# Kotstantinovskiy/SonicDiffusionBayesLab

Measured on AMD Instinct MI355X. Metric: 512x512 images/sec at 50 DDIM steps, higher is better.
Workload: dtype bf16; 1 GPU; SD-1.5 512x512 DDIM 50 steps, CFG 7.5, batch=8/GPU (BASELINE configs[1]); global_batch=8, sample_size=64, parallelism=batch-shard x1, weights=SD-1.5-shaped synthetic seed 1234

## Files before the change

include/sd_hip.h:

```cpp
#ifndef SD_HIP_H
#define SD_HIP_H

#ifdef __cplusplus
extern "C" {
#endif

typedef struct sd_unet sd_unet;

typedef struct sd_unet_config {
    int sample_size;
    int in_channels;
    int out_channels;
    int num_levels;
    int block_out_channels[8];
    int layers_per_block;
    int attn_levels[8];
    int cross_attention_dim;
    int num_heads;
    int norm_num_groups;
    float norm_eps;
    int context_len;
    int weight_dtype;
    float fp8_act_scale_norm;
    float fp8_act_scale_ff;
// ... 126 lines not shown
int sd_unet_debug_tensor(sd_unet* u, void* stream, const char* name, float* host_out, long long numel,
                         void* workspace, int unet_batch, int cache_branch_id);

int sd_sched_step(void* stream, const float* eps, int cfg, float guidance, const float* x, const float* m1,
                  const float* m2, const float* m3, const float* noise, float* prev, float* y2, float* m_out,
                  const float coef[10], long long n);

int sd_cfg_rescale_factors(void* stream, const float* eps, int batch, long long n_per_sample, float guidance,
                           float rescale, float* k_out);
int sd_sched_step_rescaled(void* stream, const float* eps, int cfg, float guidance, const float* x, const float* m1,
                           const float* m2, const float* m3, const float* noise, float* prev, float* y2, float* m_out,
                           const float coef[10], long long n, const float* k, long long n_per_sample);

int sd_sched_step_inpaint(void* stream, const float* eps, int cfg, float guidance, const float* x, const float* m1,
                          const float* m2, const float* m3, const float* noise, float* prev, float* y2, float* m_out,
                          const float coef[10], long long n, const float* k, long long n_per_sample, const float* init,
                          const float* blend_noise, const float* mask, float a, float s, long long hw);
int sd_inpaint_prepare(void* stream, const float* image, const float* mask, float* masked_image, float* latent_mask,
                       int batch, int height, int width);

int sd_op_gemm(void* stream, const void* X, long long ldx, const void* X2, long long ldx2, int K1, const void* W,
               const float* bias, const float* bias2, const void* R, long long ldr, void* C, long long ldc, int M,
               int N, int K, int epi);
int sd_op_gemm_batched(void* stream, const void* X, long long ldx, const void* W, long long w_batch_stride,
                       int rows_per_batch, const float* bias, const void* R, long long ldr, void* C, long long ldc,
                       int M, int N, int K, int epi, int sm_valid);
int sd_op_gemm_batched_softmax_ln(void* stream, const void* X, long long ldx, const void* W, long long w_batch_stride,
                                  int rows_per_batch, void* C, long long ldc, int M, int N, int K, int sm_valid,
                                  const float* rowstats, int parts, const float* c1, const float* c2, float eps);
int sd_op_conv3x3(void* stream, const void* X, const void* W, const float* bias, const float* bias2, const void* R,
                  void* Y, int B, int Hin, int Win, int Cin, int Cout, int stride, int upsample);
int sd_op_conv3x3_shortcut(void* stream, const void* X, const void* W, const float* bias, const void* Xs1, int Cs1,
                           const void* Xs2, int Cs2, const void* Wsc, void* Y, int B, int H, int Wd, int Cin, int Cout);
int sd_op_conv3x3_shortcut_groupnorm(void* stream, const void* X, const void* W, const float* bias, const void* Xs1, int Cs1,
                                     const void* Xs2, int Cs2, const void* Wsc, void* Y, int B, int H, int Wd, int Cin,
                                     int Cout, const float* gamma, const float* beta, void* Yn, int groups, float eps, int silu);
int sd_op_conv3x3_down_asym(void* stream, const void* X, const void* W, const float* bias, void* Y, int B, int Hin, int Win,
                            int Cin, int Cout);
int sd_op_conv3x3_kernel(int M, int N, int Cin, int Hin, int Win, int stride, int upsample, int dtype);
int sd_op_softmax_rows(void* stream, void* S, long long rows, int cols, float scale);
int sd_op_conv3x3_upsample_subpixel(void* stream, const void* X, const void* W4, const float* bias, void* Y, int B, int Hin,
                                    int Win, int Cin, int Cout);
int sd_op_conv3x3_upsample_subpixel_groupnorm(void* stream, const void* X, const void* W4, const float* bias, void* Y, int B,
                                              int Hin, int Win, int Cin, int Cout, const float* gamma, const float* beta,
                                              void* Yn, int groups, float eps, int silu);
int sd_op_groupnorm(void* stream, const void* x1, int C1, const void* x2, int C2, const float* gamma,
                    const float* beta, void* y, int B, int HW, int groups, float eps, int silu);
int sd_op_conv3x3_groupnorm(void* stream, const void* X, const void* W, const float* bias, const float* bias2,
                            const void* R, void* Y, int B, int Hin, int Win, int Cin, int Cout, const float* gamma,
                            const float* beta, void* Yn, int groups, float eps, int silu);
int sd_op_conv3x3_splitk(int M, int Cout, int Cin, int Hin, int Win, int stride, int upsample);
int sd_op_layernorm(void* stream, const void* x, const float* gamma, const float* beta, void* y, int rows, int C,
                    float eps);
int sd_op_attention(void* stream, const void* Q, long long ldq, const void* K, long long ldk, const void* V,
                    long long ldv, void* O, long long ldo, int B, int heads, int Nq, int Nk, int D, float scale);
int sd_op_gemm_qkv_headmajor(void* stream, const void* X, long long ldx, const void* W, void* Q, void* KV, int M, int C,
                             int tokens, int K);
int sd_op_attention_headmajor(void* stream, const void* Q, long long ldq, const void* K, const void* V, void* O,
                              long long ldo, int B, int heads, int Nq, int Nk, int D, float scale);
int sd_op_clip_attention(void* stream, const void* qkv, void* out, int B, int L, int H, int heads);
int sd_op_vit_attention(void* stream, const void* qkv, void* out, int B, int L, int H, int heads);
int sd_op_clip_preprocess(void* stream, const unsigned char* images, int B, int H, int W, int S, int P, unsigned char* crop,
                          void* patches);
int sd_op_conv_in(void* stream, const float* x, int Bsrc, const float* Wt, const float* bias, void* y, int B, int H,
                  int W, int Cin, int Cout);
int sd_op_conv_in_cond(void* stream, const float* x, int Bsrc, const float* cond, int Bcond, const float* Wt,
                       const float* bias, void* y, int B, int H, int W, int Cout);
int sd_op_conv_out(void* stream, const void* x, const void* Wp, const float* bias, float* y, int B, int H, int W,
                   int Cin, int Cout);
int sd_op_time_embedding(void* stream, float t, const void* W1, const float* b1, const void* W2, const float* b2,
                         float* scratch, float* temb, int dim_in, int dim);
int sd_op_timestep_cond(void* stream, float t, const float* cond, const void* Wc, float* row, float* emb, int cond_dim,
                        int dim);

int sd_op_ln_partials(int kind, int M, int N);
int sd_op_gemm_rowstats(void* stream, const void* X, long long ldx, const void* W, const float* bias, const void* R,
                        long long ldr, void* C, long long ldc, int M, int N, int K, float* rowstats);
int sd_op_gemm_ln(void* stream, const void* X, long long ldx, const void* Wg, const float* c1, const float* c2,
                  const float* rowstats, int parts, float eps, void* C, long long ldc, int M, int N, int K, int epi);
int sd_op_gemm_plan(void* stream, const void* X, long long ldx, const void* X2, long long ldx2, int K1, const void* W,
                    const float* bias, const float* bias2, const void* R, long long ldr, void* C, long long ldc, int M, int N,
                    int K, float* rowstats, float* stats, const float* ln_rs, int ln_parts, const float* ln_c1, float ln_eps,
                    void* KV, int hm_tokens);
int sd_op_xattn_fused_rowstats(void* stream, const void* X, const void* R, void* Y, const void* At, const void* Bw,
                               const float* bias, int M, int C, int rows_per_sample, int L, float* rowstats);
int sd_op_xattn_fused(void* stream, const void* X, const void* R, void* Y, const void* At, const void* Bw,
                      const float* bias, int M, int C, int rows_per_sample, int L);
int sd_op_xattn_fused_ln(void* stream, const void* X, const void* R, void* Y, const void* At, const void* Bw,
                         const float* bias, int M, int C, int rows_per_sample, int L, const float* ln_rowstats, int ln_parts,
                         long long ln_rows, const float* c2, float eps, float* rowstats);
int sd_op_conv3x3_ablate(void* stream, const void* X, const void* W, void* Y, int B, int Hin, int Win, int Cin, int Cout,
                         int ablate);
int sd_op_xattn_fused_stamps(void* stream, const void* X, const void* R, void* Y, const void* At, const void* Bw,
                             const float* bias, int M, int C, int rows_per_sample, int L, unsigned long long* stamps);

int sd_op_gemm_fp8(void* stream, const void* X, long long ldx, const void* W, const float* wscale, float xscale,
                   const float* bias, const void* R, long long ldr, void* C, long long ldc, int M, int N, int K, int epi,
                   int out_fp8, float oscale);
int sd_op_conv3x3_fp8(void* stream, const void* X, const void* W, const float* wscale, float xscale, const float* bias,
                      const float* bias2, const void* R, void* Y, int B, int Hin, int Win, int Cin, int Cout, int stride,
                      int upsample);
int sd_op_groupnorm_fp8(void* stream, const void* x1, int C1, const void* x2, int C2, const float* gamma,
                        const float* beta, void* y, int B, int HW, int groups, float eps, int silu, int Cpad, float oscale);
int sd_op_layernorm_fp8(void* stream, const void* x, const float* gamma, const float* beta, void* y, int rows, int C,
                        int Cpad, float eps, float oscale);
int sd_op_quantize_fp8(void* stream, const void* x_bf16, void* y_fp8, long long rows, int C, int Cpad, float scale);
int sd_op_amax_e4m3(void* stream, const void* codes, long long nbytes, unsigned* out_code);

#ifdef __cplusplus
}
#endif
#endif
```

sonicdiffusionbayeslab_amd/_lib.py:

```python
from __future__ import annotations

import ctypes as C
import os
import re
from typing import Optional

HERE = os.path.dirname(os.path.abspath(__file__))
LIB_PATH = os.environ.get("SD_AMD_LIB", os.path.join(HERE, "lib", "libsdhip.so"))
HEADER_PATH = os.path.normpath(os.path.join(HERE, "..", "include", "sd_hip.h"))

ABLATE_LIB_PATH = os.path.join(HERE, "lib", "libsdhip_ablate.so")

_lib: Optional[C.CDLL] = None
_ablate: Optional[C.CDLL] = None


class SdUnetConfig(C.Structure):
    _fields_ = [
        ("sample_size", C.c_int), ("in_channels", C.c_int), ("out_channels", C.c_int),
        ("num_levels", C.c_int), ("block_out_channels", C.c_int * 8), ("layers_per_block", C.c_int),
        ("attn_levels", C.c_int * 8), ("cross_attention_dim", C.c_int), ("num_heads", C.c_int),
        ("norm_num_groups", C.c_int), ("norm_eps", C.c_float), ("context_len", C.c_int),
        ("weight_dtype", C.c_int), ("fp8_act_scale_norm", C.c_float), ("fp8_act_scale_ff", C.c_float),
        ("time_cond_proj_dim", C.c_int),
# ... 43 lines not shown
    "sd_unet_fp8_scale_count": (_i, [_vp]),
    "sd_unet_fp8_scale_info": (_i, [_vp, _i, C.c_char_p, _i, C.POINTER(_f), C.POINTER(_f)]),
    "sd_unet_set_fp8_scale": (_i, [_vp, C.c_char_p, _f]),
    "sd_unet_workspace_bytes": (_ll, [_vp, _i, _i]),
    "sd_unet_set_context": (_i, [_vp, _vp, _vp, _i, _i, _vp, _ll]),
    "sd_unet_set_timestep_cond": (_i, [_vp, _vp, _vp]),
    "sd_unet_forward": (_i, [_vp, _vp, _vp, _i, _i, _f, _vp, _vp, _ll, _i, _i]),
    "sd_unet_workspace_bytes_hw": (_ll, [_vp, _i, _i, _i, _i]),
    "sd_unet_set_context_hw": (_i, [_vp, _vp, _vp, _i, _i, _i, _i, _vp, _ll]),
    "sd_unet_forward_hw": (_i, [_vp, _vp, _vp, _i, _i, _i, _i, _f, _vp, _vp, _ll, _i, _i]),
    "sd_unet_forward_profiled": (_i, [_vp, _vp, _vp, _i, _i, _f, _vp, _vp, _ll, _i, _i, C.POINTER(C.c_double),
                                      C.POINTER(_ll), C.POINTER(C.c_double), C.POINTER(C.c_double)]),
    "sd_unet_forward_op_times": (_ll, [_vp, _vp, _vp, _i, _i, _f, _vp, _vp, _ll, _i, _i, C.c_char_p, _ll]),
    "sd_vae_create": (_i, [C.POINTER(SdUnetConfig), C.POINTER(_vp)]),
    "sd_vae_decode": (_i, [_vp, _vp, _vp, _i, _f, _vp, _vp, _ll]),
    "sd_vae_decode_hw": (_i, [_vp, _vp, _vp, _i, _i, _i, _f, _vp, _vp, _ll]),
    "sd_vae_encoder_create": (_i, [C.POINTER(SdUnetConfig), C.POINTER(_vp)]),
    "sd_vae_encode_hw": (_i, [_vp, _vp, _vp, _i, _i, _i, _vp, _vp, _ll]),
    "sd_vae_posterior_sample": (_i, [_vp, _vp, _vp, _f, _vp, _i, _ll]),
    "sd_clip_create": (_i, [C.POINTER(SdClipConfig), C.POINTER(_vp)]),
    "sd_clip_encode": (_i, [_vp, _vp, _vp, _i, _vp, _vp, _ll]),
    "sd_clip_create_projected": (_i, [C.POINTER(SdClipConfig), _i, _i, C.POINTER(_vp)]),
    "sd_clip_text_embeds_workspace_bytes": (_ll, [_vp, _i]),
    "sd_clip_text_embeds": (_i, [_vp, _vp, _vp, _i, _vp, _vp, _ll]),
    "sd_clip_vision_create": (_i, [C.POINTER(SdClipVisionConfig), C.POINTER(_vp)]),
    "sd_clip_vision_workspace_bytes": (_ll, [_vp, _i, _i, _i]),
    "sd_clip_vision_encode": (_i, [_vp, _vp, _vp, _i, _i, _i, _vp, _vp, _ll]),
    "sd_clip_score": (_i, [_vp, _vp, _vp, _i, _i, _vp, _vp]),
    "sd_clip_resize_taps": (_i, [_i, _i, _i, _i, _vp, _vp, _vp]),
    "sd_op_vit_attention": (_i, [_vp, _vp, _vp, _i, _i, _i, _i]),
    "sd_op_clip_preprocess": (_i, [_vp, _vp, _i, _i, _i, _i, _i, _vp, _vp]),
    "sd_inception_create": (_i, [C.POINTER(_vp)]),
    "sd_inception_destroy": (None, [_vp]),
    "sd_inception_num_convs": (_i, [_vp]),
    "sd_inception_conv_info": (_i, [_vp, _i, C.c_char_p, _i, C.POINTER(_ll)]),
    "sd_inception_load_conv": (_i, [_vp, C.c_char_p, _vp, _ll, _vp, _i]),
    "sd_inception_finalize": (_i, [_vp]),
    "sd_inception_workspace_bytes": (_ll, [_vp, _i, _i]),
    "sd_inception_features": (_i, [_vp, _vp, _vp, _i, _i, _i, _i, _vp, _vp, _ll]),
    "sd_fid_accumulate": (_i, [_vp, _vp, _i, _i, _vp, _vp, _vp]),
    "sd_op_inception_conv": (_i, [_vp, _vp, _vp, _vp, _vp, _i, _i, _i, _i, _i, _i, _i, _i, _i, _i, _i, _i, _i]),
    "sd_op_maxpool3x3": (_i, [_vp, _vp, _vp, _i, _i, _i, _i, _i, _i, _i, _i]),
    "sd_op_avgpool3x3": (_i, [_vp, _vp, _vp, _i, _i, _i, _i, _i, _i]),
    "sd_op_global_mean": (_i, [_vp, _vp, _vp, _i, _i, _i]),
    "sd_op_inception_resize": (_i, [_vp, _vp, _i, _i, _i, _vp, _i]),
    "sd_unet_debug_tensor": (_i, [_vp, _vp, C.c_char_p, _vp, _ll, _vp, _i, _i]),
    "sd_sched_step": (_i, [_vp, _vp, _i, _f, _vp, _vp, _vp, _vp, _vp, _vp, _vp, _vp, C.POINTER(_f), _ll]),
    "sd_cfg_rescale_factors": (_i, [_vp, _vp, _i, _ll, _f, _f, _vp]),
    "sd_sched_step_rescaled": (_i, [_vp, _vp, _i, _f, _vp, _vp, _vp, _vp, _vp, _vp, _vp, _vp, C.POINTER(_f), _ll, _vp, _ll]),
    "sd_sched_step_inpaint": (_i, [_vp, _vp, _i, _f, _vp, _vp, _vp, _vp, _vp, _vp, _vp, _vp, C.POINTER(_f), _ll, _vp, _ll,
                                   _vp, _vp, _vp, _f, _f, _ll]),
    "sd_inpaint_prepare": (_i, [_vp, _vp, _vp, _vp, _vp, _i, _i, _i]),
    "sd_unet_set_inpaint_cond_hw": (_i, [_vp, _vp, _vp, _vp, _i, _i, _i]),
    "sd_op_conv_in_cond": (_i, [_vp, _vp, _i, _vp, _i, _vp, _vp, _vp, _i, _i, _i, _i]),
    "sd_op_gemm": (_i, [_vp, _vp, _ll, _vp, _ll, _i, _vp, _vp, _vp, _vp, _ll, _vp, _ll, _i, _i, _i, _i]),
    "sd_op_gemm_batched": (_i, [_vp, _vp, _ll, _vp, _ll, _i, _vp, _vp, _ll, _vp, _ll, _i, _i, _i, _i, _i]),
    "sd_op_gemm_batched_softmax_ln": (_i, [_vp, _vp, _ll, _vp, _ll, _i, _vp, _ll, _i, _i, _i, _i, _vp, _i, _vp, _vp, _f]),
    "sd_op_conv3x3": (_i, [_vp, _vp, _vp, _vp, _vp, _vp, _vp, _i, _i, _i, _i, _i, _i, _i]),
    "sd_op_conv3x3_shortcut": (_i, [_vp, _vp, _vp, _vp, _vp, _i, _vp, _i, _vp, _vp, _i, _i, _i, _i, _i]),
    "sd_op_conv3x3_shortcut_groupnorm": (_i, [_vp, _vp, _vp, _vp, _vp, _i, _vp, _i, _vp, _vp, _i, _i, _i, _i, _i,
                                              _vp, _vp, _vp, _i, _f, _i]),
    "sd_op_conv3x3_down_asym": (_i, [_vp, _vp, _vp, _vp, _vp, _i, _i, _i, _i, _i]),
    "sd_op_conv3x3_ablate": (_i, [_vp, _vp, _vp, _vp, _i, _i, _i, _i, _i, _i]),
    "sd_op_conv3x3_upsample_subpixel": (_i, [_vp, _vp, _vp, _vp, _vp, _i, _i, _i, _i, _i]),
    "sd_op_conv3x3_upsample_subpixel_groupnorm": (_i, [_vp, _vp, _vp, _vp, _vp, _i, _i, _i, _i, _i, _vp, _vp, _vp, _i, _f, _i]),
    "sd_op_groupnorm": (_i, [_vp, _vp, _i, _vp, _i, _vp, _vp, _vp, _i, _i, _i, _f, _i]),
    "sd_op_conv3x3_groupnorm": (_i, [_vp, _vp, _vp, _vp, _vp, _vp, _vp, _i, _i, _i, _i, _i, _vp, _vp, _vp, _i, _f, _i]),
    "sd_op_conv3x3_splitk": (_i, [_i, _i, _i, _i, _i, _i, _i]),
    "sd_op_conv3x3_kernel": (_i, [_i, _i, _i, _i, _i, _i, _i, _i]),
    "sd_op_softmax_rows": (_i, [_vp, _vp, _ll, _i, _f]),
    "sd_op_layernorm": (_i, [_vp, _vp, _vp, _vp, _vp, _i, _i, _f]),
    "sd_op_attention": (_i, [_vp, _vp, _ll, _vp, _ll, _vp, _ll, _vp, _ll, _i, _i, _i, _i, _i, _f]),
    "sd_op_gemm_qkv_headmajor": (_i, [_vp, _vp, _ll, _vp, _vp, _vp, _i, _i, _i, _i]),
    "sd_op_attention_headmajor": (_i, [_vp, _vp, _ll, _vp, _vp, _vp, _ll, _i, _i, _i, _i, _i, _f]),
    "sd_op_clip_attention": (_i, [_vp, _vp, _vp, _i, _i, _i, _i]),
    "sd_op_conv_in": (_i, [_vp, _vp, _i, _vp, _vp, _vp, _i, _i, _i, _i, _i]),
    "sd_op_conv_out": (_i, [_vp, _vp, _vp, _vp, _vp, _i, _i, _i, _i, _i]),
    "sd_op_time_embedding": (_i, [_vp, _f, _vp, _vp, _vp, _vp, _vp, _vp, _i, _i]),
    "sd_op_timestep_cond": (_i, [_vp, _f, _vp, _vp, _vp, _vp, _i, _i]),
    "sd_op_ln_partials": (_i, [_i, _i, _i]),
    "sd_op_gemm_rowstats": (_i, [_vp, _vp, _ll, _vp, _vp, _vp, _ll, _vp, _ll, _i, _i, _i, _vp]),
    "sd_op_gemm_plan": (_i, [_vp, _vp, _ll, _vp, _ll, _i, _vp, _vp, _vp, _vp, _ll, _vp, _ll, _i, _i, _i, _vp, _vp, _vp, _i, _vp, _f,
                            _vp, _i]),
    "sd_op_gemm_ln": (_i, [_vp, _vp, _ll, _vp, _vp, _vp, _vp, _i, _f, _vp, _ll, _i, _i, _i, _i]),
    "sd_op_xattn_fused_rowstats": (_i, [_vp, _vp, _vp, _vp, _vp, _vp, _vp, _i, _i, _i, _i, _vp]),
    "sd_op_xattn_fused": (_i, [_vp, _vp, _vp, _vp, _vp, _vp, _vp, _i, _i, _i, _i]),
    "sd_op_xattn_fused_ln": (_i, [_vp, _vp, _vp, _vp, _vp, _vp, _vp, _i, _i, _i, _i, _vp, _i, _ll, _vp, _f, _vp]),
    "sd_op_xattn_fused_stamps": (_i, [_vp, _vp, _vp, _vp, _vp, _vp, _vp, _i, _i, _i, _i, _vp]),
    "sd_op_gemm_fp8": (_i, [_vp, _vp, _ll, _vp, _vp, _f, _vp, _vp, _ll, _vp, _ll, _i, _i, _i, _i, _i, _f]),
    "sd_op_conv3x3_fp8": (_i, [_vp, _vp, _vp, _vp, _f, _vp, _vp, _vp, _vp, _i, _i, _i, _i, _i, _i, _i]),
    "sd_op_groupnorm_fp8": (_i, [_vp, _vp, _i, _vp, _i, _vp, _vp, _vp, _i, _i, _i, _f, _i, _i, _f]),
    "sd_op_layernorm_fp8": (_i, [_vp, _vp, _vp, _vp, _vp, _i, _i, _i, _f, _f]),
    "sd_op_quantize_fp8": (_i, [_vp, _vp, _vp, _ll, _i, _i, _f]),
    "sd_op_amax_e4m3": (_i, [_vp, _vp, _ll, _vp]),
}


def load() -> C.CDLL:
    global _lib
    if _lib is not None:
        return _lib
    if not os.path.exists(LIB_PATH):
        raise SdHipError(
            f"{LIB_PATH} is missing: build it with `python -m sonicdiffusionbayeslab_amd.build` "
            "(or __graft_entry__.build()).  There is no CPU/PyTorch fallback for the hot path.")
    lib = C.CDLL(LIB_PATH)
    for name, (res, args) in _SIGS.items():
        fn = getattr(lib, name)
        fn.restype = res
        fn.argtypes = args
    _lib = lib
    return lib


def load_ablate() -> C.CDLL:
    global _ablate
    if _ablate is not None:
        return _ablate
    if not os.path.exists(ABLATE_LIB_PATH):
        raise SdHipError(f"{ABLATE_LIB_PATH} is missing: build it with `python -m sonicdiffusionbayeslab_amd.build`")
    lib = C.CDLL(ABLATE_LIB_PATH)
    for name, (res, args) in _SIGS.items():
        fn = getattr(lib, name)
        fn.restype = res
        fn.argtypes = args
    _ablate = lib
    return lib


def check(rc: int, what: str = "libsdhip call", lib: Optional[C.CDLL] = None) -> None:
    if rc != 0:
        msg = (lib or load()).sd_last_error()
        raise SdHipError(f"{what} failed (rc={rc}): {msg.decode() if msg else '?'}")


def ptr(t) -> Optional[int]:
    return None if t is None else t.data_ptr()


def current_stream() -> int:
    import torch
    return torch.cuda.current_stream().cuda_stream
```

sonicdiffusionbayeslab_amd/build.py:

```python
from __future__ import annotations

import os
import shutil
import subprocess
import sys
import tempfile
from concurrent.futures import ThreadPoolExecutor

HERE = os.path.dirname(os.path.abspath(__file__))
CSRC = os.path.join(HERE, "csrc")
LIB_DIR = os.path.join(HERE, "lib")
LIB_PATH = os.path.join(LIB_DIR, "libsdhip.so")
ABLATE_LIB_PATH = os.path.join(LIB_DIR, "libsdhip_ablate.so")
ABLATE_SOURCES = ("gemm_conv.hip", "conv_halo.hip")
SOURCES = ["gemm_conv.hip", "gemm_lean.hip", "conv_halo.hip", "norm.hip", "attention.hip", "xattn.hip", "small.hip", "clip.hip", "vit.hip", "inception.hip", "unet.hip"]
HEADERS = ["common.h", "kernels.h", os.path.join("..", "..", "include", "sd_hip.h")]
FLAGS = ["--offload-arch=gfx950", "-O3", "-fPIC", "-std=c++17", "-Wall", "-Wno-unused-function"]
NO_PACKED_FP32 = ["-Xclang", "-target-feature", "-Xclang", "-packed-fp32-ops"]
EXTRA_FLAGS = {"attention.hip": ["-mllvm", "-amdgpu-mfma-vgpr-form", "-ffinite-math-only", *NO_PACKED_FP32],
               "xattn.hip": ["-mllvm", "-amdgpu-mfma-vgpr-form", "-fno-slp-vectorize"],
               "small.hip": NO_PACKED_FP32, "clip.hip": NO_PACKED_FP32, "vit.hip": NO_PACKED_FP32, "norm.hip": NO_PACKED_FP32,
               "inception.hip": NO_PACKED_FP32,
               "gemm_conv.hip": ["-fno-slp-vectorize"], "gemm_lean.hip": ["-fno-slp-vectorize"]}
_HOST_NOISE = "is not a recognized feature for this target (ignoring feature)"


def _newer(a: str, b: str) -> bool:
    return (not os.path.exists(b)) or os.path.getmtime(a) > os.path.getmtime(b)


def asm_path(src: str, ablate: bool = False) -> str:
    return os.path.join(LIB_DIR, src.replace(".hip", ".ablate.s" if ablate else ".s"))


def lint_asm(path: str, unit: str, verbose: bool = True) -> None:
    from . import asm_lint
    bad = asm_lint.lint_file(path, unit, verbose=verbose)
    if bad:
        raise RuntimeError(f"{unit}: the assembly hipcc produced violates {len(bad)} rule(s) of asm_lint.py (first: {bad[0]}); "
                           "see the VIOLATION lines above and sonicdiffusionbayeslab_amd/asm_lint.py for what each rule guards")


def compile_unit(hipcc: str, src: str, obj: str, flags, verbose: bool = True) -> None:
    s = os.path.join(CSRC, src)
    tmp = tempfile.mkdtemp(prefix="sdhip_", dir=LIB_DIR)
    try:
        cmd = [hipcc, *flags, "-save-temps", "-c", s, "-o", os.path.join(tmp, "unit.o")]
        if verbose:
            print(" ".join(cmd), flush=True)
        r = subprocess.run(cmd, capture_output=True, text=True, cwd=tmp)
        err = "\n".join(l for l in r.stderr.splitlines() if _HOST_NOISE not in l and "argument unused during compilation" not in l)
        if r.returncode != 0:
            raise RuntimeError(f"hipcc failed:\n{' '.join(cmd)}\n{r.stdout}\n{err}")
        if verbose and err.strip():
            print(err, file=sys.stderr)
        dev = [f for f in os.listdir(tmp) if f.endswith("-gfx950.s")]
        if len(dev) != 1:
            raise RuntimeError(f"{src}: expected one device assembly file from -save-temps, found {dev}")
        asm = obj[:-2] + ".s"
        shutil.move(os.path.join(tmp, dev[0]), asm)
        try:
            lint_asm(asm, src.split(".")[0], verbose=verbose)
        except Exception:
            os.replace(asm, asm + ".rejected")
            raise
        shutil.move(os.path.join(tmp, "unit.o"), obj)
    finally:
        shutil.rmtree(tmp, ignore_errors=True)


def build_library(force: bool = False, verbose: bool = True) -> str:
    hipcc = os.environ.get("HIPCC", "/opt/rocm/bin/hipcc")
    if not os.path.exists(hipcc):
        hipcc = "hipcc"
    os.makedirs(LIB_DIR, exist_ok=True)
    hdrs = [os.path.normpath(os.path.join(CSRC, h)) for h in HEADERS]
    me = [os.path.abspath(__file__), os.path.join(HERE, "asm_lint.py")]
    objs, jobs = [], []
    for src in SOURCES:
        s = os.path.join(CSRC, src)
        o = os.path.join(LIB_DIR, src.replace(".hip", ".o"))
        objs.append(o)
        if force or _newer(s, o) or any(_newer(h, o) for h in hdrs + me) or not os.path.exists(o[:-2] + ".s"):
            jobs.append((src, o, [*FLAGS, *EXTRA_FLAGS.get(src, [])]))

    aobjs, ajobs = [], []
    for src in SOURCES:
        s = os.path.join(CSRC, src)
        if src in ABLATE_SOURCES:
            o = os.path.join(LIB_DIR, src.replace(".hip", ".ablate.o"))
            if force or _newer(s, o) or any(_newer(h, o) for h in hdrs + me) or not os.path.exists(o[:-2] + ".s"):
                ajobs.append((src, o, [*FLAGS, "-DSD_ABLATE", *EXTRA_FLAGS.get(src, [])]))
        else:
            o = os.path.join(LIB_DIR, src.replace(".hip", ".o"))
        aobjs.append(o)

    def run(cmd):
        if verbose:
            print(" ".join(cmd), flush=True)
# ... 16 lines not shown
```

sonicdiffusionbayeslab_amd/csrc/gemm_lean.hip:

```cpp
#include "common.h"
#include "kernels.h"
#include <mutex>
#include <stdlib.h>

namespace {

typedef __amdgpu_buffer_rsrc_t rsrc_t;

struct LeanArgs {
    const void* X; const void* X2; const void* W; const void* R; void* C; void* KV;
    const float* vec0; const float* vec1;
    const float* ln_rs; float* rowstats; float* stats;
    unsigned x_bytes, x2_bytes, w_bytes, r_bytes, c_bytes, kv_bytes;
    int M, N, K, K1;
    int ldxb, ldx2b, ldwb, ldrb, ldcb;
    int tiles_m, tiles_n;
    float ln_eps, inv_k;
    int hm_tpc;
    int hm_tok_shift, hm_heads, hm_samples;
};

template <int N>
__device__ __forceinline__ void wait_vmcnt() {
    asm volatile("s_waitcnt vmcnt(%0)" ::"n"(N) : "memory");
}

__device__ __forceinline__ rsrc_t make_rsrc(const void* p, unsigned bytes) {
    return __builtin_amdgcn_make_buffer_rsrc((void*)p, 0, (int)bytes, 0x00020000);
}
__device__ __forceinline__ void dma16(rsrc_t r, void* lds_wave_base, int voff, int soff) {
    __builtin_amdgcn_raw_ptr_buffer_load_lds(r, LDS_PTR(lds_wave_base), 16, voff, soff, 0, 0);
}

template <int BM, int BN, int WAVES_M, int WAVES_N, int NP, bool GEGLU>
__global__ __launch_bounds__(WAVES_M* WAVES_N * 64, 2) void gemm_lean_kernel(const LeanArgs p) {
    constexpr bool LN = NP > 0;
    constexpr int NW = WAVES_M * WAVES_N;
    constexpr int WTM = BM / WAVES_M, WTN = BN / WAVES_N;
    constexpr int TM = WTM / 16, TN = WTN / 16;
    constexpr int XI = BM / 8, WI = BN / 8;
    static_assert(XI % NW == 0 && WI % NW == 0, "pieces split evenly over the waves");
    constexpr int XPW = XI / NW, WPW = WI / NW;
    constexpr int STAGE_BYTES = (BM + BN) * 128;
    static_assert(GEGLU ? TN % 4 == 0 : TN % 2 == 1, "store schedule: GEGLU pairs of output tiles; std TN / 2 paired + one 8-byte store");
    constexpr bool FRAG_DB = TM * TN * 4 + (TM + TN) * 8 <= 200;
    constexpr int TNH = GEGLU ? TN / 2 : TN;

    extern __shared__ __attribute__((aligned(16))) char smem[];
    char* lnbuf = smem + 2 * STAGE_BYTES;
    char* vecs = lnbuf + NW * 512;

    const int tid = threadIdx.x, lane = tid & 63;
    const int wave = __builtin_amdgcn_readfirstlane(tid >> 6);
    const int wm = wave % WAVES_M, wn = wave / WAVES_M;
    const int lrow = lane & 15, lq = lane >> 4;

    const int nblk = gridDim.x;
    int work;
    {
        const int q = nblk >> 3, r = nblk & 7, xcd = blockIdx.x & 7, idx = blockIdx.x >> 3;
        work = (xcd < r ? xcd * (q + 1) : r * (q + 1) + (xcd - r) * q) + idx;
    }
    const int nwork = p.tiles_m * p.tiles_n;
    if (work >= nwork) return;
    int tile_m = work / p.tiles_n, tile_n = work - tile_m * p.tiles_n;
    const int dm = nblk / p.tiles_n, dn = nblk - dm * p.tiles_n;

    const rsrc_t rX = make_rsrc(p.X, p.x_bytes), rW = make_rsrc(p.W, p.w_bytes), rC = make_rsrc(p.C, p.c_bytes);
    const rsrc_t rX2 = make_rsrc(LN ? p.X : p.X2, LN ? 0 : p.x2_bytes), rR = make_rsrc(LN ? p.X : p.R, LN ? 0 : p.r_bytes);
    const rsrc_t rKV = make_rsrc(LN ? p.KV : p.C, LN ? p.kv_bytes : 0);

    const int lrow8 = lane >> 3, gch = (lane & 7) ^ lrow8;
    const int vX = lrow8 * p.ldxb + gch * 16, vX2 = lrow8 * p.ldx2b + gch * 16, vW = lrow8 * p.ldwb + gch * 16;
    const int rowl = wm * WTM + lrow;
    const int vR = rowl * p.ldrb + (wn * WTN + lq * 4) * 2;
    const int vCw = rowl * p.ldcb + (wn * WTN + (lq & 1) * 16 + (lq >> 1) * 8) * 2;
    const int vCn = rowl * p.ldcb + (wn * WTN + lq * 4) * 2;
    const int vCg = rowl * p.ldcb + (wn * WTN / 2 + (lq & 1) * 16 + (lq >> 1) * 8) * 2;
    int vH[TN / 2 + 1] = {};
#pragma unroll
    for (int j = 0; LN && !GEGLU && j <= TN / 2; ++j) {
        const int cl = wn * WTN + (j < TN / 2 ? j * 32 + (lq & 1) * 16 + (lq >> 1) * 8 : (TN - 1) * 16 + lq * 4);
        const int hl = (cl * 205) >> 13;
        vH[j] = ((hl << p.hm_tok_shift) + rowl) * 80 + (cl - hl * 40) * 2;
    }
    const int vLn = (wm * WTM + lane) * 8;
    const int vRs = rowl * 8;
    const int vSt = (wn * WTN + lq * 4) * 8;
    const int vVec = (wn * WTN + lane * 4) * 4;

    const int swz[2] = {((lq) ^ (lane & 7)) << 4, ((4 + lq) ^ (lane & 7)) << 4};
    const int xoff = (wm * WTM + lrow) * 128;
    const int woff = BM * 128 + (wn * WTN + lrow) * 128;

    const int KT = p.K >> 6;
    int m0 = tile_m * BM, n0 = tile_n * BN;

    auto stage = [&](int kt, int buf) {
        char* xs = smem + buf * STAGE_BYTES;
        char* ws = xs + BM * 128;
        const int k0 = kt * 64;
        if (LN || k0 < p.K1) {
            const int so = (m0 + wave * 8) * p.ldxb + k0 * 2;
#pragma unroll
            for (int i = 0; i < XPW; ++i) dma16(rX, xs + (wave + i * NW) * 1024, vX, so + i * (NW * 8) * p.ldxb);
        } else {
            const int so = (m0 + wave * 8) * p.ldx2b + (k0 - p.K1) * 2;
#pragma unroll
            for (int i = 0; i < XPW; ++i) dma16(rX2, xs + (wave + i * NW) * 1024, vX2, so + i * (NW * 8) * p.ldx2b);
        }
        const int sw = (n0 + wave * 8) * p.ldwb + k0 * 2;
#pragma unroll
        for (int i = 0; i < WPW; ++i) dma16(rW, ws + (wave + i * NW) * 1024, vW, sw + i * (NW * 8) * p.ldwb);
    };

    f32x4 acc[TN][TM];
    bf16x8 xf0[TM], wf0[TN], xf1[FRAG_DB ? TM : 1], wf1[FRAG_DB ? TN : 1];
    auto load_frags = [&](const char* sb, int ks, bf16x8* xf, bf16x8* wf) {
#pragma unroll
        for (int t = 0; t < TM; ++t) xf[t] = *(const bf16x8*)(sb + xoff + t * 2048 + swz[ks]);
#pragma unroll
        for (int t = 0; t < TN; ++t) wf[t] = *(const bf16x8*)(sb + woff + t * 2048 + swz[ks]);
    };
    auto mfmas = [&](const bf16x8* xf, const bf16x8* wf) {
#pragma unroll
        for (int a = 0; a < TN; ++a)
#pragma unroll
            for (int b = 0; b < TM; ++b)
                acc[a][b] = __builtin_amdgcn_mfma_f32_16x16x32_bf16(wf[a], xf[b], acc[a][b], 0, 0, 0);
    };

    constexpr int EPI_STORES = GEGLU ? (TN / 4) * TM : (TN / 2 + 1) * TM;
    int g = 0;
    bool stores_pending = false;
    stage(0, 0);
    while (true) {
#pragma unroll
        for (int a = 0; a < TN; ++a)
#pragma unroll
            for (int b = 0; b < TM; ++b) acc[a][b] = f32x4{0.f, 0.f, 0.f, 0.f};
        for (int kt = 0; kt < KT - 1; ++kt) {
            if (kt == 0 && stores_pending) wait_vmcnt<EPI_STORES>();
            else wait_vmcnt<0>();
            __builtin_amdgcn_s_barrier();
            asm volatile("" ::: "memory");
            const char* sb = smem + ((g + kt) & 1) * STAGE_BYTES;
            load_frags(sb, 0, xf0, wf0);
            __builtin_amdgcn_sched_barrier(0);
            stage(kt + 1, (g + kt + 1) & 1);
// ... 21 lines not shown
            const char* sb = smem + ((g + KT - 1) & 1) * STAGE_BYTES;
            load_frags(sb, 0, xf0, wf0);
            if (FRAG_DB) load_frags(sb, 1, xf1, wf1);
            if (LN) {
                const char* src = (const char*)p.ln_rs + (long)m0 * 8;
#pragma unroll
                for (int i = 0; i < NP; ++i) ep[i] = *(const u32x2*)((src + (long)i * p.M * 8) + (unsigned)vLn);
            } else if (!GEGLU && p.R) {
                const int so = m0 * p.ldrb + n0 * 2;
#pragma unroll
                for (int b = 0; b < TM; ++b)
#pragma unroll
                    for (int a = 0; a < TN; ++a)
                        ep[a * TM + b] = __builtin_bit_cast(u32x2, __builtin_amdgcn_raw_buffer_load_b64(rR, vR + a * 32, so + b * 16 * p.ldrb, 0));
            }
            __builtin_amdgcn_sched_barrier(0);
            mfmas(xf0, wf0);
            if (FRAG_DB) {
                mfmas(xf1, wf1);
            } else {
                load_frags(sb, 1, xf0, wf0);
                mfmas(xf0, wf0);
            }
            __builtin_amdgcn_sched_barrier(0);
        }
        g += KT;

        f32x4 v0[TNH], v1[TNH];
        auto vec_load = [&](int a0) {
#pragma unroll
            for (int a = 0; a < TNH; ++a) {
                v0[a] = *(const f32x4*)(vecs + (wn * WTN + (a0 + a) * 16 + lq * 4) * 4);
                v1[a] = *(const f32x4*)(vecs + BN * 4 + (wn * WTN + (a0 + a) * 16 + lq * 4) * 4);
            }
        };
        vec_load(0);
        if (LN) {
            float s = 0.f, q = 0.f;
#pragma unroll
            for (int i = 0; i < NP; ++i) {
                const f32x2_t e = __builtin_bit_cast(f32x2_t, ep[i]);
                s += e[0];
                q += e[1];
            }
            *(f32x2_t*)(lnbuf + wave * 512 + lane * 8) = ln_mean_rstd(s, q, p.inv_k, p.ln_eps);
            f32x2_t mr[TM];
#pragma unroll
            for (int b = 0; b < TM; ++b) mr[b] = *(const f32x2_t*)(lnbuf + wave * 512 + (b * 16 + lrow) * 8);
#pragma unroll
            for (int a0 = 0; a0 < TN; a0 += TNH) {
                if (a0 > 0) vec_load(a0);
#pragma unroll
                for (int a = 0; a < TNH; ++a)
#pragma unroll
                    for (int b = 0; b < TM; ++b) acc[a0 + a][b] = ln_fold(acc[a0 + a][b], v0[a], mr[b][0], mr[b][1], v1[a]);
            }
        } else {
            if (!GEGLU && p.R) {
#pragma unroll
                for (int a = 0; a < TN; ++a)
#pragma unroll
                    for (int b = 0; b < TM; ++b) {
                        const u32x2 r = ep[a * TM + b];
                        acc[a][b][0] += bflo(r[0]); acc[a][b][1] += bfhi(r[0]);
                        acc[a][b][2] += bflo(r[1]); acc[a][b][3] += bfhi(r[1]);
                    }
            }
#pragma unroll
            for (int a0 = 0; a0 < TN; a0 += TNH) {
                if (a0 > 0) vec_load(a0);
#pragma unroll
                for (int a = 0; a < TNH; ++a) {
                    const f32x4 bv = v0[a] + v1[a];
#pragma unroll
                    for (int b = 0; b < TM; ++b) acc[a0 + a][b] += bv;
                }
            }
        }

        const int em0 = m0, en0 = n0, etile_n = tile_n;
        work += nblk;
        const bool more = work < nwork;
        if (more) {
            tile_n += dn; tile_m += dm;
            if (tile_n >= p.tiles_n) { tile_n -= p.tiles_n; tile_m += 1; }
            m0 = tile_m * BM; n0 = tile_n * BN;
            stage(0, g & 1);
            stores_pending = true;
        }

        if (!LN && !GEGLU && WTM == 64 && p.stats) {
            char* dst = (char*)p.stats + ((long)((em0 + wm * WTM) >> 6) * p.N + en0) * 8 + (unsigned)vSt;
#pragma unroll
            for (int a = 0; a < TN; ++a) {
                float sv[4] = {0.f, 0.f, 0.f, 0.f}, qv[4] = {0.f, 0.f, 0.f, 0.f};
#pragma unroll
                for (int b = 0; b < TM; ++b) {
                    const unsigned p0 = pack2bf(acc[a][b][0], acc[a][b][1]), p1 = pack2bf(acc[a][b][2], acc[a][b][3]);
                    const float v[4] = {bflo(p0), bfhi(p0), bflo(p1), bfhi(p1)};
#pragma unroll
                    for (int j = 0; j < 4; ++j) { sv[j] += v[j]; qv[j] = __builtin_fmaf(v[j], v[j], qv[j]); }
                }
#pragma unroll
                for (int j = 0; j < 4; ++j) {
                    sv[j] = row_shr_add<8>(row_shr_add<4>(row_shr_add<2>(row_shr_add<1>(sv[j]))));
                    qv[j] = row_shr_add<8>(row_shr_add<4>(row_shr_add<2>(row_shr_add<1>(qv[j]))));
                }
                if (lrow == 15) {
                    *(f32x4*)(dst + a * 128) = f32x4{sv[0], qv[0], sv[1], qv[1]};
                    *(f32x4*)(dst + a * 128 + 16) = f32x4{sv[2], qv[2], sv[3], qv[3]};
                }
            }
        }
        if (!LN && !GEGLU && p.rowstats) {
            char* dst = (char*)p.rowstats + ((long)(etile_n * WAVES_N + wn) * p.M + em0) * 8 + (unsigned)vRs;
#pragma unroll
            for (int b = 0; b < TM; ++b) {
                float s = 0.f, q = 0.f;
#pragma unroll
                for (int a = 0; a < TN; ++a) {
                    const unsigned p0 = pack2bf(acc[a][b][0], acc[a][b][1]), p1 = pack2bf(acc[a][b][2], acc[a][b][3]);
                    const float v[4] = {bflo(p0), bfhi(p0), bflo(p1), bfhi(p1)};
#pragma unroll
                    for (int j = 0; j < 4; ++j) { s += v[j]; q = __builtin_fmaf(v[j], v[j], q); }
                }
                s += __shfl_xor(s, 16); q += __shfl_xor(q, 16);
                s += __shfl_xor(s, 32); q += __shfl_xor(q, 32);
                if (lq == 0) *(f32x2_t*)(dst + b * 16 * 8) = f32x2_t{s, q};
            }
        }
        if constexpr (GEGLU) {
            auto geglu_tile = [&](int a, int b) -> u32x2 {
                const f32x4 va = acc[a][b], vg = acc[a + 1][b];
                const f32x2_t lo = geglu_pair(f32x2_t{va[0], va[1]}, f32x2_t{vg[0], vg[1]});
                const f32x2_t hi = geglu_pair(f32x2_t{va[2], va[3]}, f32x2_t{vg[2], vg[3]});
                return u32x2{pack2bf(lo[0], lo[1]), pack2bf(hi[0], hi[1])};
            };
            const int soC = em0 * p.ldcb + en0;
#pragma unroll
            for (int b = 0; b < TM; ++b) {
                const int vo = vCg + (soC + b * 16 * p.ldcb);
#pragma unroll
                for (int a = 0; a < TN; a += 4) {
                    const u32x2 ox = geglu_tile(a, b), oy = geglu_tile(a + 2, b);
                    const auto s0 = __builtin_amdgcn_permlane16_swap(ox[0], oy[0], false, false);
                    const auto s1 = __builtin_amdgcn_permlane16_swap(ox[1], oy[1], false, false);
                    __builtin_amdgcn_raw_buffer_store_b128(u32x4{s0[0], s1[0], s0[1], s1[1]}, rC, vo + a * 16, 0, 0);
                }
            }
        } else {
            u32x4 ow[TM][TN / 2];
            u32x2 on[TM];
#pragma unroll
            for (int b = 0; b < TM; ++b) {
#pragma unroll
                for (int a = 0; a + 1 < TN; a += 2) {
                    const f32x4 vx = acc[a][b], vy = acc[a + 1][b];
                    const auto s0 = __builtin_amdgcn_permlane16_swap(pack2bf(vx[0], vx[1]), pack2bf(vy[0], vy[1]), false, false);
                    const auto s1 = __builtin_amdgcn_permlane16_swap(pack2bf(vx[2], vx[3]), pack2bf(vy[2], vy[3]), false, false);
                    ow[b][a / 2] = u32x4{s0[0], s1[0], s0[1], s1[1]};
                }
                const f32x4 v = acc[TN - 1][b];
                on[b] = u32x2{pack2bf(v[0], v[1]), pack2bf(v[2], v[3])};
            }
            if (LN && p.hm_tpc > 0 && etile_n >= p.hm_tpc) {
                const int which = etile_n >= 2 * p.hm_tpc ? 1 : 0;
                const int head0 = (etile_n - (which + 1) * p.hm_tpc) * 4;
                const int smp = em0 >> p.hm_tok_shift, tok0 = em0 & ((1 << p.hm_tok_shift) - 1);
                const int soC = ((((which * p.hm_samples + smp) * p.hm_heads + head0) << p.hm_tok_shift) + tok0) * 80;
#pragma unroll
                for (int b = 0; b < TM; ++b) {
                    const int so = soC + b * 16 * 80;
#pragma unroll
                    for (int j = 0; j < TN / 2; ++j) __builtin_amdgcn_raw_buffer_store_b128(ow[b][j], rKV, vH[j] + so, 0, 0);
                    __builtin_amdgcn_raw_buffer_store_b64(on[b], rKV, vH[TN / 2] + so, 0, 0);
                }
            } else {
                const int soC = em0 * p.ldcb + en0 * 2;
#pragma unroll
                for (int b = 0; b < TM; ++b) {
                    const int so = soC + b * 16 * p.ldcb;
#pragma unroll
                    for (int j = 0; j < TN / 2; ++j) __builtin_amdgcn_raw_buffer_store_b128(ow[b][j], rC, vCw + so + j * 64, 0, 0);
                    __builtin_amdgcn_raw_buffer_store_b64(on[b], rC, vCn + so + (TN - 1) * 32, 0, 0);
                }
            }
        }
        if (!more) break;
    }
}

static const float* zero_vector() {
    static std::mutex mu;
    static float* z[16] = {};
    int dev = 0;
    if (hipGetDevice(&dev) != hipSuccess || dev < 0 || dev >= 16) return nullptr;
    std::lock_guard<std::mutex> lock(mu);
    if (!z[dev]) {
        float* p = nullptr;
        float probe = 1.f;
        if (hipMalloc((void**)&p, 16384 * 4) != hipSuccess) return nullptr;
        if (hipMemset(p, 0, 16384 * 4) != hipSuccess || hipMemcpy(&probe, p + 16383, 4, hipMemcpyDeviceToHost) != hipSuccess || probe != 0.f) {
            (void)hipFree(p);
            return nullptr;
        }
        z[dev] = p;
    }
    return z[dev];
}

template <int BM, int BN, int WAVES_M, int WAVES_N, int NP, bool GEGLU>
int launch_lean(const LeanArgs& a0, hipStream_t stream) {
    LeanArgs a = a0;
    a.tiles_m = (a.M + BM - 1) / BM;
    a.tiles_n = a.N / BN;
    constexpr int NW = WAVES_M * WAVES_N;
    constexpr int smem = 2 * (BM + BN) * 128 + NW * 512 + 2 * BN * 4;
    static_assert(smem <= 160 * 1024, "tile does not fit the 160 KiB LDS");
    auto kern = gemm_lean_kernel<BM, BN, WAVES_M, WAVES_N, NP, GEGLU>;
    static bool attr_set = false;
    if (!attr_set) {
        SD_CHECK_HIP(hipFuncSetAttribute((const void*)kern, hipFuncAttributeMaxDynamicSharedMemorySize, smem));
        attr_set = true;
    }
    int grid = a.tiles_m * a.tiles_n;
    constexpr int resident = smem > 80 * 1024 ? 256 : 512;
    if (grid > resident) grid = resident;
    hipLaunchKernelGGL(kern, dim3(grid), dim3(NW * 64), smem, stream, a);
    SD_CHECK_HIP(hipGetLastError());
    return 0;
}

}

bool sd_gemm_lean_applicable(const GemmArgs& a, int epi) {
    if ((epi != 0 && epi != 1) || a.dt != 0 || a.out_fp8 || a.rows_per_batch || a.subpix || (a.splitk > 1 && a.slab)) return false;
    const int BN = epi ? 256 : 160;
    if (a.N % BN != 0 || a.N > 16384 || a.K % 64 != 0 || a.K < 128 || a.K1 % 64 != 0 || a.M < 1) return false;
    if (a.K1 != a.K && a.X2 == nullptr) return false;
    if ((a.ldc & 7) || (a.ldx & 7) || (a.X2 && (a.ldx2 & 7)) || (a.ldw & 7) || (a.R && (a.ldr & 3))) return false;
    const long big = 1L << 31;
    const long ldw = a.ldw ? a.ldw : a.K;
    if ((long)a.M * a.ldx * 2 >= big || (long)a.M * a.ldc * 2 >= big || (long)a.N * ldw * 2 >= big) return false;
    if (a.X2 && (long)a.M * a.ldx2 * 2 >= big) return false;
    if (a.R && (long)a.M * a.ldr * 2 >= big) return false;
    if ((a.stats || a.rowstats || a.ln_rs || a.hm_C) && a.M % (epi ? 256 : 128) != 0) return false;
    if (a.ln_rs) {
        if (a.R || a.bias2 || !a.bias || !a.ln_c1 || a.X2 || a.K1 != a.K || a.stats || a.rowstats) return false;
        if (a.ln_np != 2 && a.ln_np != 4 && a.ln_np != 8 && a.ln_np != 16) return false;
    }
    if (epi == 1 && (a.R || a.bias2 || a.X2 || a.K1 != a.K || a.stats || a.rowstats || a.hm_C)) return false;
    if (a.hm_C) {
        if (!a.ln_rs || !a.KV || a.hm_C % 160 != 0 || a.N != 3 * a.hm_C || a.hm_tok < 128 || (a.hm_tok & (a.hm_tok - 1)) ||
            a.M % a.hm_tok != 0 || (long)a.M * a.hm_C * 4 >= big)
            return false;
    }
    return true;
}

int sd_launch_gemm_lean(const GemmArgs& g, int epi, int rows, hipStream_t stream) {
    SD_REQUIRE(sd_gemm_lean_applicable(g, epi), "gemm (lean): problem not supported (M=%d N=%d K=%d epi=%d)", g.M, g.N, g.K, epi);
    SD_REQUIRE(epi == 1 || rows == 128 || (rows == 64 && !g.stats && !g.ln_rs && !g.hm_C),
               "gemm (lean): %d-row tile with block statistics / LayerNorm fold / head-major K|V", rows);
    const long ldw = g.ldw ? g.ldw : g.K;
    LeanArgs a{};
    a.X = g.X; a.X2 = g.X2; a.W = g.W; a.R = g.R; a.C = g.C; a.KV = g.KV;
    a.M = g.M; a.N = g.N; a.K = g.K; a.K1 = g.K1;
    a.ldxb = (int)g.ldx * 2; a.ldx2b = (int)g.ldx2 * 2; a.ldwb = (int)ldw * 2; a.ldrb = (int)g.ldr * 2; a.ldcb = (int)g.ldc * 2;
    a.x_bytes = (unsigned)(((long)g.M - 1) * g.ldx * 2 + (long)g.K1 * 2);
    a.x2_bytes = g.X2 ? (unsigned)(((long)g.M - 1) * g.ldx2 * 2 + (long)(g.K - g.K1) * 2) : 0;
    a.w_bytes = (unsigned)(((long)g.N - 1) * ldw * 2 + (long)g.K * 2);
    a.r_bytes = g.R ? (unsigned)(((long)g.M - 1) * g.ldr * 2 + (long)g.N * 2) : 0;
    const int ncols = epi ? g.N / 2 : g.hm_C ? g.hm_C : g.N;
    a.c_bytes = (unsigned)(((long)g.M - 1) * g.ldc * 2 + (long)ncols * 2);
    a.kv_bytes = g.hm_C ? (unsigned)((long)g.M * g.hm_C * 4) : 0;
    const float* zeros = nullptr;
    if (!g.bias || (!g.ln_rs && !g.bias2)) {
        zeros = zero_vector();
        SD_REQUIRE(zeros, "gemm (lean): cannot allocate the zero vector");
    }
    if (g.ln_rs) {
        a.vec0 = g.ln_c1; a.vec1 = g.bias; a.ln_rs = g.ln_rs; a.ln_eps = g.ln_eps; a.inv_k = 1.0f / (float)g.K;
    } else {
        a.vec0 = g.bias ? g.bias : zeros; a.vec1 = g.bias2 ? g.bias2 : zeros;
    }
    a.rowstats = g.rowstats; a.stats = g.stats;
    if (g.hm_C) {
        a.hm_tpc = g.hm_C / 160;
        int sh = 0;
        while ((1 << sh) < g.hm_tok) ++sh;
        a.hm_tok_shift = sh; a.hm_heads = g.hm_C / 40; a.hm_samples = g.M / g.hm_tok;
    }
    if (epi == 1) {
        if (!g.ln_rs) return launch_lean<256, 256, 4, 2, 0, true>(a, stream);
        return g.ln_np == 2 ? launch_lean<256, 256, 4, 2, 2, true>(a, stream)
             : g.ln_np == 4 ? launch_lean<256, 256, 4, 2, 4, true>(a, stream)
             : g.ln_np == 8 ? launch_lean<256, 256, 4, 2, 8, true>(a, stream) : launch_lean<256, 256, 4, 2, 16, true>(a, stream);
    }
    if (g.ln_rs)
        return g.ln_np == 2 ? launch_lean<128, 160, 2, 2, 2, false>(a, stream)
             : g.ln_np == 4 ? launch_lean<128, 160, 2, 2, 4, false>(a, stream)
             : g.ln_np == 8 ? launch_lean<128, 160, 2, 2, 8, false>(a, stream) : launch_lean<128, 160, 2, 2, 16, false>(a, stream);
    return rows == 64 ? launch_lean<64, 160, 2, 2, 0, false>(a, stream) : launch_lean<128, 160, 2, 2, 0, false>(a, stream);
}
```

Baseline: 11.62 images/s.

## Remap lean GEMM persistent tile order into XCD-aware rectangles for cache reuse

Replaces the row-major persistent-tile walk in the lean GEMM kernel with a configurable mapping. It groups tiles into a×b rectangles per group of eight workgroups, which matches the eight-XCD layout, so co-resident workgroups share X and W panels in L2. A host-side chooser picks the rectangle shape with a cost model. The mapping is skipped for small weight matrices and can be overridden via SD_GEMM_RECT. Each tile now needs extra magic-number divisions, and the rectangle parameters are read from kernarg memory.

```diff
diff --git a/include/sd_hip.h b/include/sd_hip.h
--- a/include/sd_hip.h
+++ b/include/sd_hip.h
@@ -232,6 +232,8 @@
                     const float* bias, const float* bias2, const void* R, long long ldr, void* C, long long ldc, int M, int N,
                     int K, float* rowstats, float* stats, const float* ln_rs, int ln_parts, const float* ln_c1, float ln_eps,
                     void* KV, int hm_tokens);
+int sd_op_gemm_order_table(int tiles_m, int tiles_n, int grid, int a, int b, int m_fast, int* tiles);
+int sd_op_gemm_order_choose(int M, int N, int K, int epi, int rows, int* grid, int* a, int* b, int* m_fast);
 int sd_op_xattn_fused_rowstats(void* stream, const void* X, const void* R, void* Y, const void* At, const void* Bw,
                                const float* bias, int M, int C, int rows_per_sample, int L, float* rowstats);
 int sd_op_xattn_fused(void* stream, const void* X, const void* R, void* Y, const void* At, const void* Bw,
diff --git a/sonicdiffusionbayeslab_amd/_lib.py b/sonicdiffusionbayeslab_amd/_lib.py
--- a/sonicdiffusionbayeslab_amd/_lib.py
+++ b/sonicdiffusionbayeslab_amd/_lib.py
@@ -149,6 +149,8 @@
     "sd_op_gemm_rowstats": (_i, [_vp, _vp, _ll, _vp, _vp, _vp, _ll, _vp, _ll, _i, _i, _i, _vp]),
     "sd_op_gemm_plan": (_i, [_vp, _vp, _ll, _vp, _ll, _i, _vp, _vp, _vp, _vp, _ll, _vp, _ll, _i, _i, _i, _vp, _vp, _vp, _i, _vp, _f,
                             _vp, _i]),
+    "sd_op_gemm_order_table": (_i, [_i, _i, _i, _i, _i, _i, _vp]),
+    "sd_op_gemm_order_choose": (_i, [_i, _i, _i, _i, _i, C.POINTER(_i), C.POINTER(_i), C.POINTER(_i), C.POINTER(_i)]),
     "sd_op_gemm_ln": (_i, [_vp, _vp, _ll, _vp, _vp, _vp, _vp, _i, _f, _vp, _ll, _i, _i, _i, _i]),
     "sd_op_xattn_fused_rowstats": (_i, [_vp, _vp, _vp, _vp, _vp, _vp, _vp, _i, _i, _i, _i, _vp]),
     "sd_op_xattn_fused": (_i, [_vp, _vp, _vp, _vp, _vp, _vp, _vp, _i, _i, _i, _i]),
diff --git a/sonicdiffusionbayeslab_amd/build.py b/sonicdiffusionbayeslab_amd/build.py
--- a/sonicdiffusionbayeslab_amd/build.py
+++ b/sonicdiffusionbayeslab_amd/build.py
@@ -14,7 +14,7 @@
 ABLATE_LIB_PATH = os.path.join(LIB_DIR, "libsdhip_ablate.so")
 ABLATE_SOURCES = ("gemm_conv.hip", "conv_halo.hip")
 SOURCES = ["gemm_conv.hip", "gemm_lean.hip", "conv_halo.hip", "norm.hip", "attention.hip", "xattn.hip", "small.hip", "clip.hip", "vit.hip", "inception.hip", "unet.hip"]
-HEADERS = ["common.h", "kernels.h", os.path.join("..", "..", "include", "sd_hip.h")]
+HEADERS = ["common.h", "kernels.h", "gemm_order.h", os.path.join("..", "..", "include", "sd_hip.h")]
 FLAGS = ["--offload-arch=gfx950", "-O3", "-fPIC", "-std=c++17", "-Wall", "-Wno-unused-function"]
 NO_PACKED_FP32 = ["-Xclang", "-target-feature", "-Xclang", "-packed-fp32-ops"]
 EXTRA_FLAGS = {"attention.hip": ["-mllvm", "-amdgpu-mfma-vgpr-form", "-ffinite-math-only", *NO_PACKED_FP32],
diff --git a/sonicdiffusionbayeslab_amd/csrc/gemm_lean.hip b/sonicdiffusionbayeslab_amd/csrc/gemm_lean.hip
--- a/sonicdiffusionbayeslab_amd/csrc/gemm_lean.hip
+++ b/sonicdiffusionbayeslab_amd/csrc/gemm_lean.hip
@@ -1,6 +1,10 @@
 #include "common.h"
 #include "kernels.h"
+#include "gemm_order.h"
+#include "../../include/sd_hip.h"
 #include <mutex>
+#include <stddef.h>
+#include <stdio.h>
 #include <stdlib.h>
 
 namespace {
@@ -15,6 +19,7 @@
     int M, N, K, K1;
     int ldxb, ldx2b, ldwb, ldrb, ldcb;
     int tiles_m, tiles_n;
+    GemmOrder ord;
     float ln_eps, inv_k;
     int hm_tpc;
     int hm_tok_shift, hm_heads, hm_samples;
@@ -63,8 +68,19 @@
     }
     const int nwork = p.tiles_m * p.tiles_n;
     if (work >= nwork) return;
-    int tile_m = work / p.tiles_n, tile_n = work - tile_m * p.tiles_n;
-    const int dm = nblk / p.tiles_n, dn = nblk - dm * p.tiles_n;
+    int tile_m, tile_n;
+    auto decode = [&](int w) {
+#if defined(__HIP_DEVICE_COMPILE__)
+        typedef const __attribute__((address_space(4))) char* kernarg_t;
+        int off = (int)(offsetof(LeanArgs, ord) + offsetof(GemmOrder, r));
+        asm volatile("" : "+s"(off));
+        sd_gemm_order_map(p.ord, (const __attribute__((address_space(4))) GemmOrderRect*)((kernarg_t)__builtin_amdgcn_kernarg_segment_ptr() + off),
+                          (unsigned)w, &tile_m, &tile_n);
+#else
+        sd_gemm_order_map(p.ord, &p.ord.r, (unsigned)w, &tile_m, &tile_n);
+#endif
+    };
+    decode(work);
 
     const rsrc_t rX = make_rsrc(p.X, p.x_bytes), rW = make_rsrc(p.W, p.w_bytes), rC = make_rsrc(p.C, p.c_bytes);
     const rsrc_t rX2 = make_rsrc(LN ? p.X : p.X2, LN ? 0 : p.x2_bytes), rR = make_rsrc(LN ? p.X : p.R, LN ? 0 : p.r_bytes);
@@ -252,8 +268,7 @@
         work += nblk;
         const bool more = work < nwork;
         if (more) {
-            tile_n += dn; tile_m += dm;
-            if (tile_n >= p.tiles_n) { tile_n -= p.tiles_n; tile_m += 1; }
+            decode(work);
             m0 = tile_m * BM; n0 = tile_n * BN;
             stage(0, g & 1);
             stores_pending = true;
@@ -379,6 +394,28 @@
     return z[dev];
 }
 
+static int lean_grid(int items, bool geglu) {
+    const int resident = geglu ? 256 : 512;
+    return items < resident ? items : resident;
+}
+
+static bool lean_order_gated(int N, int K) { return (long)N * K * 2 < 8L << 20; }
+
+static void lean_order(int tiles_m, int tiles_n, int bm, int bn, int grid, int N, int K, int* a, int* b, int* m_fast) {
+    sd_gemm_order_choose(tiles_m, tiles_n, bm, bn, grid, a, b, m_fast);
+    if (lean_order_gated(N, K)) *a = *b = *m_fast = 0;
+    const char* env = getenv("SD_GEMM_RECT");
+    int ea = 0, eb = 0, n;
+    char dir = 0;
+    if (env && (n = sscanf(env, "%dx%d%c", &ea, &eb, &dir)) >= 2) {
+        const bool fits = (grid & 7) == 0 && ea > 0 && eb > 0 && ea * eb == grid >> 3 && ea <= tiles_m && eb <= tiles_n;
+        *a = fits ? ea : 0; *b = fits ? eb : 0;
+        *m_fast = n == 3 && (dir == 'm' || dir == 'n') ? dir == 'm' : (long)eb * bn >= (long)ea * bm;
+    } else if (env && atoi(env) == 0) {
+        *a = *b = *m_fast = 0;
+    }
+}
+
 template <int BM, int BN, int WAVES_M, int WAVES_N, int NP, bool GEGLU>
 int launch_lean(const LeanArgs& a0, hipStream_t stream) {
     LeanArgs a = a0;
@@ -387,15 +424,17 @@
     constexpr int NW = WAVES_M * WAVES_N;
     constexpr int smem = 2 * (BM + BN) * 128 + NW * 512 + 2 * BN * 4;
     static_assert(smem <= 160 * 1024, "tile does not fit the 160 KiB LDS");
+    static_assert((smem > 80 * 1024) == GEGLU, "lean_grid: one workgroup per CU for the GEGLU tile, two for the others");
     auto kern = gemm_lean_kernel<BM, BN, WAVES_M, WAVES_N, NP, GEGLU>;
     static bool attr_set = false;
     if (!attr_set) {
         SD_CHECK_HIP(hipFuncSetAttribute((const void*)kern, hipFuncAttributeMaxDynamicSharedMemorySize, smem));
         attr_set = true;
     }
-    int grid = a.tiles_m * a.tiles_n;
-    constexpr int resident = smem > 80 * 1024 ? 256 : 512;
-    if (grid > resident) grid = resident;
+    const int grid = lean_grid(a.tiles_m * a.tiles_n, GEGLU);
+    int ra, rb, rmf;
+    lean_order(a.tiles_m, a.tiles_n, BM, BN, grid, a.N, a.K, &ra, &rb, &rmf);
+    a.ord = sd_gemm_order_make(a.tiles_m, a.tiles_n, grid, ra, rb, rmf);
     hipLaunchKernelGGL(kern, dim3(grid), dim3(NW * 64), smem, stream, a);
     SD_CHECK_HIP(hipGetLastError());
     return 0;
@@ -473,3 +512,25 @@
              : g.ln_np == 8 ? launch_lean<128, 160, 2, 2, 8, false>(a, stream) : launch_lean<128, 160, 2, 2, 16, false>(a, stream);
     return rows == 64 ? launch_lean<64, 160, 2, 2, 0, false>(a, stream) : launch_lean<128, 160, 2, 2, 0, false>(a, stream);
 }
+
+extern "C" int sd_op_gemm_order_table(int tiles_m, int tiles_n, int grid, int a, int b, int m_fast, int* tiles) {
+    if (tiles_m < 1 || tiles_n < 1 || grid < 1 || !tiles) return -1;
+    const GemmOrder o = sd_gemm_order_make(tiles_m, tiles_n, grid, a, b, m_fast);
+    for (int w = 0; w < tiles_m * tiles_n; ++w) {
+        int tm = -1, tn = -1;
+        sd_gemm_order_map(o, &o.r, (unsigned)w, &tm, &tn);
+        tiles[2 * w] = tm; tiles[2 * w + 1] = tn;
+    }
+    return 0;
+}
+
+extern "C" int sd_op_gemm_order_choose(int M, int N, int K, int epi, int rows, int* grid, int* a, int* b, int* m_fast) {
+    if (M < 1 || N < 1 || K < 1 || (epi != 0 && epi != 1) || (epi == 0 && rows != 64 && rows != 128) || !grid || !a || !b || !m_fast)
+        return -1;
+    const int bm = epi ? 256 : rows, bn = epi ? 256 : 160;
+    if (N % bn != 0) return -1;
+    const int tiles_m = (M + bm - 1) / bm, tiles_n = N / bn;
+    *grid = lean_grid(tiles_m * tiles_n, epi == 1);
+    sd_gemm_order_choose(tiles_m, tiles_n, bm, bn, *grid, a, b, m_fast);
+    return *a != 0 && lean_order_gated(N, K) ? 1 : 0;
+}
diff --git a/sonicdiffusionbayeslab_amd/csrc/gemm_order.h b/sonicdiffusionbayeslab_amd/csrc/gemm_order.h
--- /dev/null
+++ b/sonicdiffusionbayeslab_amd/csrc/gemm_order.h
@@ -0,0 +1,104 @@
+#pragma once
+
+#ifndef __host__
+#define __host__
+#define __device__
+#endif
+
+struct GemmOrderDiv {
+    unsigned mul, shift;
+};
+inline GemmOrderDiv sd_gemm_order_div(unsigned d) {
+    GemmOrderDiv f = {0u, 0u};
+    if (d == 0) return f;
+    while ((1ull << f.shift) < d) ++f.shift;
+    f.mul = (unsigned)((((1ull << f.shift) - d) << 32) / d) + 1u;
+    return f;
+}
+__host__ __device__ inline unsigned sd_gemm_order_quot(unsigned n, GemmOrderDiv f) {
+    return ((unsigned)(((unsigned long long)n * f.mul) >> 32) + n) >> f.shift;
+}
+
+struct GemmOrderRect {
+    unsigned b, m_fast;
+    unsigned q, nrq;
+    unsigned base, rem;
+    unsigned run;
+    unsigned row0, col0, cn, top;
+    GemmOrderDiv dq, db, drun, dcn;
+};
+struct GemmOrder {
+    unsigned a;
+    unsigned tiles_n;
+    GemmOrderDiv dtn;
+    GemmOrderRect r;
+};
+
+inline GemmOrder sd_gemm_order_make(int tiles_m, int tiles_n, int grid, int a, int b, int m_fast) {
+    GemmOrder o = {};
+    o.tiles_n = (unsigned)tiles_n;
+    o.dtn = sd_gemm_order_div(o.tiles_n);
+    const int q = grid >> 3;
+    if ((grid & 7) != 0 || a <= 0 || b <= 0 || (long)a * b != q || a > tiles_m || b > tiles_n) return o;
+    const unsigned rm_n = tiles_m / a, rn_n = tiles_n / b, nr = rm_n * rn_n;
+    GemmOrderRect& r = o.r;
+    o.a = a; r.b = b; r.m_fast = m_fast ? 1 : 0;
+    r.q = q; r.nrq = nr * q;
+    r.base = nr >> 3; r.rem = nr & 7;
+    r.run = m_fast ? rm_n : rn_n;
+    r.row0 = rm_n * a; r.col0 = rn_n * b; r.cn = tiles_n - r.col0; r.top = r.row0 * r.cn;
+    r.dq = sd_gemm_order_div(r.q); r.db = sd_gemm_order_div(r.b); r.drun = sd_gemm_order_div(r.run); r.dcn = sd_gemm_order_div(r.cn);
+    return o;
+}
+
+template <class R>
+__host__ __device__ inline void sd_gemm_order_map(const GemmOrder& o, R rp, unsigned w, int* tile_m, int* tile_n) {
+    if (o.a != 0) {
+        const GemmOrderRect r = *rp;
+        if (w < r.nrq) {
+            const unsigned k = sd_gemm_order_quot(w, r.dq), i = w - k * r.q;
+            const unsigned x = k & 7, t = x * r.base + (x < r.rem ? x : r.rem) + (k >> 3);
+            const unsigned hi = sd_gemm_order_quot(t, r.drun), lo = t - hi * r.run;
+            const unsigned im = sd_gemm_order_quot(i, r.db);
+            *tile_m = (int)((r.m_fast ? lo : hi) * o.a + im);
+            *tile_n = (int)((r.m_fast ? hi : lo) * r.b + (i - im * r.b));
+            return;
+        }
+        const unsigned w2 = w - r.nrq;
+        if (w2 < r.top) {
+            const unsigned m = sd_gemm_order_quot(w2, r.dcn);
+            *tile_m = (int)m;
+            *tile_n = (int)(r.col0 + (w2 - m * r.cn));
+            return;
+        }
+        w = w2 - r.top;
+        const unsigned m = sd_gemm_order_quot(w, o.dtn);
+        *tile_m = (int)(r.row0 + m);
+        *tile_n = (int)(w - m * o.tiles_n);
+        return;
+    }
+    const unsigned m = sd_gemm_order_quot(w, o.dtn);
+    *tile_m = (int)m;
+    *tile_n = (int)(w - m * o.tiles_n);
+}
+
+inline void sd_gemm_order_choose(int tiles_m, int tiles_n, int bm, int bn, int grid, int* a_out, int* b_out, int* m_fast) {
+    *a_out = *b_out = *m_fast = 0;
+    const int q = grid >> 3;
+    if ((grid & 7) != 0 || q < 2 || tiles_m < 1 || tiles_n < 1) return;
+    const long total = (long)tiles_m * tiles_n;
+    const long present = (long)((q + tiles_n - 1) / tiles_n) * bm + (long)(q < tiles_n ? q : tiles_n) * bn;
+    long best = -1;
+    int ba = 0, bb = 0;
+    for (int a = 1; a <= q; ++a) {
+        if (q % a != 0) continue;
+        const int b = q / a;
+        if (a > tiles_m || b > tiles_n) continue;
+        const long in = (long)(tiles_m / a) * a * (tiles_n / b) * b;
+        const long cost = in * ((long)a * bm + (long)b * bn) + (total - in) * present;
+        if (best < 0 || cost < best) { best = cost; ba = a; bb = b; }
+    }
+    if (best < 0 || (present * total - best) * 4 < present * total) return;
+    *a_out = ba; *b_out = bb;
+    *m_fast = (long)bb * bn >= (long)ba * bm ? 1 : 0;
+}
```

New measurement: 11.62 images/s (median of 3 runs). Within noise of the previous version (+0.0%).
